# alessandroragano/nomad

Measured on AMD Instinct MI355X. Metric: clips/sec embedded + NxM NOMAD distances, 16kHz x 4s batches, higher is better.
Workload: dtype f32; 1 GPU; configs[1]: batch=256 x 64000 samples (T=199) per GPU, wav2vec2-base + projection head fp32, 224 deg x 32*N ref float64 distances + means; deg_per_gpu=224, ref_total=32, parallelism=clip-sharded x1, all-gather of ref embeddings, collective=none (single process, no process group)

## Files before the change

include/nomad_hip.h:

```cpp
#ifndef NOMAD_HIP_H
#define NOMAD_HIP_H

#include <stddef.h>
#include <stdint.h>

#ifdef __cplusplus
extern "C" {
#endif

#define NOMAD_NUM_LAYERS 12
#define NOMAD_EMBED_DIM 768
#define NOMAD_EMB_DIM 256

typedef enum nomad_status {
    NOMAD_OK = 0,
    NOMAD_ERR_INVALID = -1,
    NOMAD_ERR_NO_DEVICE = -2,
    NOMAD_ERR_HIP = -3,
    NOMAD_ERR_WORKSPACE = -4,
    NOMAD_ERR_IO = -5,
    NOMAD_ERR_FORMAT = -6
} nomad_status;

typedef struct nomad_ctx nomad_ctx;
// ... 145 lines not shown
                              float* emb_dev, void* workspace_dev, size_t workspace_bytes, nomad_stream_t stream);

typedef struct nomad_wav_info {
    int sample_rate, channels, format_tag, bits;
    long long frames;
    long long data_offset;
} nomad_wav_info;
int nomad_wav_probe(const char* const* paths, int n, nomad_wav_info* info, int* status, int threads);
int nomad_wav_frames_at(const nomad_wav_info* info, int target_rate, long long* frames);
int nomad_wav_read_rows(const char* const* paths, const nomad_wav_info* info, int n, const int* row,
                        float* dst_host, long long stride, int target_rate, int* status, int threads);

enum {
    NOMAD_K_GEMM = 0,
    NOMAD_K_ATTN = 1,
    NOMAD_K_FRONT = 2,
    NOMAD_K_ROW = 3,
    NOMAD_K_PAIR = 4,
    NOMAD_K_GEMM_BIG = 5,
    NOMAD_K_GEMM_FINE = 6,
    NOMAD_K_COUNT = 7
};
int nomad_profile_enable(nomad_ctx* ctx, int on);
int nomad_profile_reset(nomad_ctx* ctx);
int nomad_profile_read(nomad_ctx* ctx, double ms[NOMAD_K_COUNT], long long launches[NOMAD_K_COUNT],
                       double flops[NOMAD_K_COUNT]);

int nomad_diag_gemm(nomad_ctx* ctx, const float* A_dev, const float* W_dev, const float* bias_dev,
                    const float* R_dev, float* C_dev, int M, int N, int K, int gelu, int tile,
                    nomad_stream_t stream);
int nomad_diag_gemm_bf16(nomad_ctx* ctx, const void* A_dev, const void* W_dev, const float* bias_dev,
                         const void* R_dev, void* C_dev, int M, int N, int K, int gelu, int tile,
                         nomad_stream_t stream);
int nomad_diag_split_bf16(nomad_ctx* ctx, const float* in_dev, void* out_dev, long long plane, long long n, int inverse,
                          nomad_stream_t stream);
int nomad_diag_gemm_bf16x3(nomad_ctx* ctx, const void* A_dev, const void* W_dev, const float* bias_dev,
                           const void* R_dev, void* C_dev, int M, int N, int K, int gelu, int out_f32,
                           nomad_stream_t stream);
int nomad_diag_attention_bf16x3(nomad_ctx* ctx, const void* qkv_dev, void* out_dev, int B, int T, int waves,
                                nomad_stream_t stream);
int nomad_diag_attention_bf16(nomad_ctx* ctx, const void* qkv_dev, void* out_dev, int B, int T, int q_has_log2e,
                              nomad_stream_t stream);
int nomad_diag_clock_probe(nomad_ctx* ctx, unsigned long long spin_ticks, unsigned long long* out_dev,
                           nomad_stream_t stream);
int nomad_diag_layernorm(nomad_ctx* ctx, const float* in_dev, const float* gamma_dev, const float* beta_dev,
                         float* out_dev, int M, int N, nomad_stream_t stream);
int nomad_diag_attention(nomad_ctx* ctx, const float* qkv_dev, float* out_dev, int B, int T, nomad_stream_t stream);
int nomad_diag_layernorm_bwd(nomad_ctx* ctx, const float* x_dev, const float* g_dev, const float* gamma_dev,
                             float* dx_dev, int M, int N, nomad_stream_t stream);
int nomad_diag_attention_bwd(nomad_ctx* ctx, const float* qkv_dev, const float* dctx_dev, float* ctx_out_dev,
                             float* lse_dev, float* dqkv_dev, int B, int T, nomad_stream_t stream);
int nomad_diag_keep_intermediates(nomad_ctx* ctx, int on);
int nomad_diag_workspace_region(const nomad_ctx* ctx, int B, int n_samples, const char* name,
                                size_t* offset, size_t* bytes);

#ifdef __cplusplus
}
#endif
#endif
```

nomad_amd/_lib.py:

```python
from __future__ import annotations

import ctypes as C
import os

NUM_LAYERS = 12
K_GEMM, K_ATTN, K_FRONT, K_ROW, K_PAIR, K_GEMM_BIG, K_GEMM_FINE, K_COUNT = 0, 1, 2, 3, 4, 5, 6, 7
KERNEL_CLASS_NAMES = ("gemm_mfma_all", "attention_mfma", "frontend", "rowwise", "pairwise_f64",
                      "gemm_mfma_256x128", "gemm_mfma_128x64")

_fp = C.c_void_p


class LayerWeights(C.Structure):
    _fields_ = [(n, _fp) for n in ("q_w", "q_b", "k_w", "k_b", "v_w", "v_b", "o_w", "o_b", "ln1_w", "ln1_b",
                                   "fc1_w", "fc1_b", "fc2_w", "fc2_b", "ln2_w", "ln2_b")]


class Weights(C.Structure):
    _fields_ = ([("conv_w", _fp * 7)] +
                [(n, _fp) for n in ("gn_w", "gn_b", "feat_ln_w", "feat_ln_b", "proj_w", "proj_b",
                                    "pos_v", "pos_g", "pos_b", "enc_ln_w", "enc_ln_b")] +
                [("layers", LayerWeights * NUM_LAYERS), ("emb_w", _fp), ("emb_b", _fp)])


# ... 58 lines not shown
    "nomad_train_enable": (C.c_int, [C.c_void_p, C.POINTER(Weights)]),
    "nomad_train_workspace_bytes": (C.c_int, [C.c_void_p, C.c_int, C.c_int, C.POINTER(C.c_size_t)]),
    "nomad_train_zero_grad": (C.c_int, [C.c_void_p, _fp]),
    "nomad_train_backward": (C.c_int, [C.c_void_p, _fp, C.c_int, C.c_int, _fp, _fp, C.c_size_t, _fp, _fp, C.c_size_t, _fp]),
    "nomad_triplet_loss": (C.c_int, [C.c_void_p, _fp, _fp, _fp, C.c_int, C.c_float, _fp, _fp, _fp, _fp, _fp]),
    "nomad_train_adam_step": (C.c_int, [C.c_void_p, C.c_float, C.c_float, C.c_double, C.c_double, C.c_float, _fp]),
    "nomad_train_read": (C.c_int, [C.c_void_p, C.c_int, _fp, _fp]),
    "nomad_train_write": (C.c_int, [C.c_void_p, C.c_int, _fp, _fp]),
    "nomad_train_set_step": (C.c_int, [C.c_void_p, C.c_longlong]),
    "nomad_train_set_frozen": (C.c_int, [C.c_void_p, C.c_int]),
    "nomad_train_set_convnet": (C.c_int, [C.c_void_p, C.c_int]),
    "nomad_train_set_branches": (C.c_int, [C.c_void_p, C.c_int, C.POINTER(C.c_uint)]),
    "nomad_train_set_stochastic": (C.c_int, [C.c_void_p, C.c_float, C.c_float, C.c_float, C.c_ulonglong, C.c_uint]),
    "nomad_enable_bf16": (C.c_int, [C.c_void_p]),
    "nomad_workspace_bytes_bf16": (C.c_int, [C.c_void_p, C.c_int, C.c_int, C.POINTER(C.c_size_t)]),
    "nomad_embed_bf16": (C.c_int, [C.c_void_p, _fp, C.c_int, C.c_int, _fp, _fp, C.c_size_t, _fp]),
    "nomad_workspace_bytes_ragged_bf16": (C.c_int, [C.c_void_p, C.c_int, C.POINTER(C.c_int), C.POINTER(C.c_size_t)]),
    "nomad_embed_ragged_bf16": (C.c_int, [C.c_void_p, _fp, C.c_int, C.c_int, C.POINTER(C.c_int), _fp, _fp, C.c_size_t, _fp]),
    "nomad_enable_bf16x3": (C.c_int, [C.c_void_p]),
    "nomad_workspace_bytes_bf16x3": (C.c_int, [C.c_void_p, C.c_int, C.c_int, C.POINTER(C.c_size_t)]),
    "nomad_embed_bf16x3": (C.c_int, [C.c_void_p, _fp, C.c_int, C.c_int, _fp, _fp, C.c_size_t, _fp]),
    "nomad_embed_layers_bf16x3": (C.c_int, [C.c_void_p, _fp, C.c_int, C.c_int, _fp, _fp, _fp, _fp, _fp, C.c_size_t, _fp]),
    "nomad_workspace_bytes_ragged_bf16x3": (C.c_int, [C.c_void_p, C.c_int, C.POINTER(C.c_int), C.POINTER(C.c_size_t)]),
    "nomad_embed_ragged_bf16x3": (C.c_int, [C.c_void_p, _fp, C.c_int, C.c_int, C.POINTER(C.c_int), _fp, _fp, C.c_size_t, _fp]),
    "nomad_diag_attention_bf16x3": (C.c_int, [C.c_void_p, _fp, _fp, C.c_int, C.c_int, C.c_int, _fp]),
    "nomad_diag_split_bf16": (C.c_int, [C.c_void_p, _fp, _fp, C.c_longlong, C.c_longlong, C.c_int, _fp]),
    "nomad_diag_gemm_bf16x3": (C.c_int, [C.c_void_p, _fp, _fp, _fp, _fp, _fp, C.c_int, C.c_int, C.c_int, C.c_int, C.c_int, _fp]),
    "nomad_diag_gemm_bf16": (C.c_int, [C.c_void_p, _fp, _fp, _fp, _fp, _fp, C.c_int, C.c_int, C.c_int, C.c_int, C.c_int, _fp]),
    "nomad_diag_attention_bf16": (C.c_int, [C.c_void_p, _fp, _fp, C.c_int, C.c_int, C.c_int, _fp]),
    "nomad_profile_enable": (C.c_int, [C.c_void_p, C.c_int]),
    "nomad_profile_reset": (C.c_int, [C.c_void_p]),
    "nomad_profile_read": (C.c_int, [C.c_void_p, C.POINTER(C.c_double), C.POINTER(C.c_longlong), C.POINTER(C.c_double)]),
    "nomad_diag_gemm": (C.c_int, [C.c_void_p, _fp, _fp, _fp, _fp, _fp, C.c_int, C.c_int, C.c_int, C.c_int, C.c_int, _fp]),
    "nomad_diag_clock_probe": (C.c_int, [C.c_void_p, C.c_ulonglong, _fp, _fp]),
    "nomad_diag_layernorm": (C.c_int, [C.c_void_p, _fp, _fp, _fp, _fp, C.c_int, C.c_int, _fp]),
    "nomad_diag_attention": (C.c_int, [C.c_void_p, _fp, _fp, C.c_int, C.c_int, _fp]),
    "nomad_diag_layernorm_bwd": (C.c_int, [C.c_void_p, _fp, _fp, _fp, _fp, C.c_int, C.c_int, _fp]),
    "nomad_diag_attention_bwd": (C.c_int, [C.c_void_p, _fp, _fp, _fp, _fp, _fp, C.c_int, C.c_int, _fp]),
    "nomad_diag_keep_intermediates": (C.c_int, [C.c_void_p, C.c_int]),
    "nomad_diag_workspace_region": (C.c_int, [C.c_void_p, C.c_int, C.c_int, C.c_char_p,
                                              C.POINTER(C.c_size_t), C.POINTER(C.c_size_t)]),
}

LIB_PATH = os.path.join(os.path.dirname(os.path.abspath(__file__)), "libnomad_hip.so")
DIAG_LIB_PATH = os.path.join(os.path.dirname(os.path.abspath(__file__)), "libnomad_diag.so")
_libs = {}


ABI_VERSION = 3


def load(diag=None):
    if diag is None:
        diag = os.environ.get("NOMAD_DIAG_LIB", "0") == "1"
    diag = bool(diag)
    if diag in _libs:
        return _libs[diag]
    path = DIAG_LIB_PATH if diag else LIB_PATH
    variant = os.environ.get("NOMAD_LIB_VARIANT")
    if variant and variant != "main":
        path = path[:-3] + f"_{variant}.so"
    if not os.path.isfile(path):
        raise RuntimeError(f"{path} is missing: build it with `python -m nomad_amd.build` "
                           "(hipcc --offload-arch=gfx950). nomad_amd has no CPU or PyTorch fallback path.")
    lib = C.CDLL(path)
    for name, (res, args) in SIGNATURES.items():
# ... 24 lines not shown
```

nomad_amd/csrc/nomad_ctx.hip.h:

```cpp
#pragma once
#include <hip/hip_runtime.h>

#include <algorithm>
#include <cmath>
#include <cstdarg>
#include <cstdio>
#include <cstdlib>
#include <cstring>
#include <atomic>
#include <mutex>
#include <string>
#include <vector>

#include "../../include/nomad_hip.h"

#include "dtypes.hip.h"
#include "gemm_f32.hip.h"

#define NOMAD_INTERNAL __attribute__((visibility("hidden")))

using namespace nomad;

inline thread_local char g_err[512] = "";

// ... 14 lines not shown
    } while (0)

constexpr int kConvK[7] = {10, 3, 3, 3, 3, 2, 2};
constexpr int kConvS[7] = {5, 2, 2, 2, 2, 2, 2};
constexpr int kSplitKLayersMaxM = 4096;
constexpr size_t kSplitKPartFloats = (size_t)4 * 512 * 64 * 64;
constexpr long long kPairScratchDoubles = 1 << 21;
constexpr int kCdistMaxD = 4096;
constexpr int kEventChunk = 8192;
const int* const kNoInts = nullptr;
const hipStream_t kNoStream = reinterpret_cast<hipStream_t>(~uintptr_t(0));

}

struct LayerDev {
    float *qkv_w, *qkv_b, *o_w, *o_b, *ln1_w, *ln1_b, *fc1_w, *fc1_b, *fc2_w, *fc2_b, *ln2_w, *ln2_b;
};


struct Tuning {
    bool splitk_lnb_fuse = true;
    bool splitk_ln_fuse = true;
    bool splitk_posconv = true;
    bool splitk_layers = true;
    bool f32_plain_epi = true;
    bool f32_lean = true, f32_direct_epi = true, f32_skew = true, f32_res_ahead = true;
    int f32_mixed = 1;
    int f32_mixed_m1 = 0;
    int f32_mixed_slots = 0;
    double f32_mixed_min = 0.05, f32_mixed_max = 0.70;
    bool f32_mixed_prefer = false;
    bool f32_quant_tile = true;
    bool f32_conv_wino = true;
    double f32_quant_penalty = 0.0;
    bool f32_longk_33 = false;
    int f32_mid_tile = 31;
    bool f32_attn_vt4 = true;
    bool f32_attn_struct_loads = false;
    bool bf16_posconv_slab = true;
    int bf16_attn_dma = 2;
    int bf16_attn_v3 = 2;
    int bf16_attn_tail = 0;
    int bf16_ln_rows = 4;
    bool bf16_conv0_mfma = true;
    bool bf16_conv0_gelu_erf = false;
    int p8_min_tiles = 256;
    bool p8_nt_stores = true;
    int p8_rpre = 3;
    bool x3_plain_epi = true;
    bool p8_three_b = true;
    int p8_n192 = 0;
    bool p9 = true;
    bool p9_res = true;
    bool p9_share = false;
    bool p9_tail_split = false;
    int p9_short = 1;
    bool attn_bwd_small = true;
    bool p9_wl = false;
    bool p9_late = true;
    int p9_skew = 0;
    int concurrent_parts = 1;
};

#ifdef NOMAD_DIAG
static void tuning_from_env(Tuning& t) {
    auto geti = [](const char* n, int d) { const char* e = getenv(n); return e ? atoi(e) : d; };
    auto getb = [](const char* n, bool d) { const char* e = getenv(n); return e ? atoi(e) != 0 : d; };
    auto getd = [](const char* n, double d) { const char* e = getenv(n); return e ? atof(e) : d; };
    t.splitk_ln_fuse = getb("NOMAD_SPLITK_LN", t.splitk_ln_fuse);
    t.splitk_posconv = getb("NOMAD_SPLITK_POSCONV", t.splitk_posconv);
    t.splitk_layers = getb("NOMAD_SPLITK_LAYERS", t.splitk_layers);
    t.f32_plain_epi = getb("NOMAD_F32_PLAIN_EPI", t.f32_plain_epi);
    t.f32_lean = getb("NOMAD_F32_LEAN", t.f32_lean);
    t.f32_direct_epi = getb("NOMAD_F32_DIRECT_EPI", t.f32_direct_epi);
    t.f32_skew = getb("NOMAD_F32_SKEW", t.f32_skew);
    t.f32_res_ahead = getb("NOMAD_F32_RES_AHEAD", t.f32_res_ahead);
    t.f32_mixed = geti("NOMAD_F32_MIXED", t.f32_mixed);
    t.f32_mixed_m1 = geti("NOMAD_F32_MIXED_M1", t.f32_mixed_m1);
    t.f32_mixed_slots = geti("NOMAD_F32_MIXED_SLOTS", t.f32_mixed_slots);
    t.f32_mixed_min = getd("NOMAD_F32_MIXED_MIN", t.f32_mixed_min);
    t.f32_mixed_max = getd("NOMAD_F32_MIXED_MAX", t.f32_mixed_max);
    t.f32_mixed_prefer = getb("NOMAD_F32_MIXED_PREFER", t.f32_mixed_prefer);
    t.f32_quant_tile = getb("NOMAD_F32_QUANT_TILE", t.f32_quant_tile);
    t.f32_conv_wino = getb("NOMAD_F32_CONV_WINO", t.f32_conv_wino);
    t.f32_quant_penalty = getd("NOMAD_F32_QUANT_PENALTY", t.f32_quant_penalty);
    t.f32_longk_33 = getb("NOMAD_F32_LONGK_33", t.f32_longk_33);
    t.f32_mid_tile = geti("NOMAD_F32_MID_TILE", t.f32_mid_tile);
    t.bf16_attn_dma = geti("NOMAD_BF16_ATTN_DMA", t.bf16_attn_dma);
    t.f32_attn_struct_loads = geti("NOMAD_F32_ATTN_STRUCT_LOADS", t.f32_attn_struct_loads) != 0;
    t.bf16_posconv_slab = geti("NOMAD_BF16_POSCONV_SLAB", t.bf16_posconv_slab) != 0;
    t.bf16_attn_v3 = geti("NOMAD_BF16_ATTN_V3", t.bf16_attn_v3);
    t.bf16_attn_tail = geti("NOMAD_BF16_ATTN_TAIL", t.bf16_attn_tail);
    t.bf16_ln_rows = geti("NOMAD_BF16_LN_ROWS", t.bf16_ln_rows);
    t.bf16_conv0_mfma = getb("NOMAD_BF16_CONV0_MFMA", t.bf16_conv0_mfma);
    t.p8_min_tiles = geti("NOMAD_BF16_8PHASE_MIN_TILES", t.p8_min_tiles);
    t.p8_nt_stores = getb("NOMAD_BF16_NT_STORES", t.p8_nt_stores);
    t.p8_rpre = geti("NOMAD_BF16_RPRE", t.p8_rpre);
    t.x3_plain_epi = getb("NOMAD_X3_PLAIN_EPI", t.x3_plain_epi);
    t.p8_three_b = getb("NOMAD_BF16_B3", t.p8_three_b);
    t.p8_n192 = geti("NOMAD_BF16_N192", t.p8_n192);
    t.p9 = getb("NOMAD_BF16_P9", t.p9);
    t.p9_tail_split = getb("NOMAD_BF16_P9_TAIL", t.p9_tail_split);
    t.p9_share = getb("NOMAD_BF16_P9_SHARE", t.p9_share);
    t.p9_res = getb("NOMAD_BF16_P9_RES", t.p9_res);
    t.p9_short = geti("NOMAD_BF16_P9_SHORT", t.p9_short);
    t.p9_skew = geti("NOMAD_BF16_P9_SKEW", t.p9_skew);
    t.p9_late = getb("NOMAD_BF16_P9_LATE", t.p9_late);
    t.p9_wl = getb("NOMAD_BF16_P9_WL", t.p9_wl);
    t.splitk_lnb_fuse = getb("NOMAD_SPLITK_LNB", t.splitk_lnb_fuse);
    t.f32_attn_vt4 = getb("NOMAD_F32_ATTN_VT4", t.f32_attn_vt4);
    t.bf16_conv0_gelu_erf = getb("NOMAD_BF16_CONV0_GELU_ERF", t.bf16_conv0_gelu_erf);
    t.attn_bwd_small = getb("NOMAD_ATTN_BWD_SMALL", t.attn_bwd_small);
}
#endif

struct nomad_ctx {
    int device = 0;
    int num_cus = 256;
    Tuning tune;
    bool keep = false;
    float* conv0_w = nullptr;
    float* conv_w[7] = {};
    float *gn_w = nullptr, *gn_b = nullptr, *fln_w = nullptr, *fln_b = nullptr;
    float *proj_w = nullptr, *proj_b = nullptr;
    float *pos_w = nullptr, *pos_b = nullptr;
    float *eln_w = nullptr, *eln_b = nullptr;
    LayerDev layers[NOMAD_NUM_LAYERS] = {};
    float *emb_w = nullptr, *emb_b = nullptr;
    float* splitk_part = nullptr;
    float* splitk_cur = nullptr;
    size_t splitk_cur_floats = 0;
    bool splitk_ok = false;
    struct PendingLn {
        const float* gamma = nullptr;
        const float* beta = nullptr;
        float* out = nullptr;
        float* out2 = nullptr;
        bool armed = false, done = false;
    } pending_ln;
    struct PendingLnBwd {
        const float* x = nullptr;
        const float* g2 = nullptr;
        const float* gamma = nullptr;
        float* out = nullptr;
        bool armed = false, done = false;
    } pending_lnb;
    std::vector<std::pair<hipStream_t, double*>> pair_scratch;
    std::mutex pair_mu;
    bool bwd_ready = false;
    float* conv_bw_even[7] = {};
    float* conv_bw_odd[7] = {};
    float* conv_bw2[7] = {};
    float* proj_wT = nullptr;
    float* pos_wb = nullptr;
    float *qkv_wT[NOMAD_NUM_LAYERS] = {}, *o_wT[NOMAD_NUM_LAYERS] = {}, *fc1_wT[NOMAD_NUM_LAYERS] = {},
          *fc2_wT[NOMAD_NUM_LAYERS] = {};
    bool bf16_ready = false;
    bf16_t* conv_w16[7] = {};
// ... 88 lines not shown
}

GemmParams dense(const float* A, int lda, const float* W, const float* bias, const float* R, float* C, int M, int N,
                 int K, int gelu) {
    GemmParams p{};
    p.A = A;
    p.amap = plain_map(M, lda);
    p.kchunk = K;
    p.kstride = 0;
    p.W = W;
    p.ldw = K;
    p.C = C;
    p.cmap = plain_map(M, N);
    p.bias = bias;
    p.R = R;
    p.rmap = plain_map(M, N);
    p.M = M;
    p.N = N;
    p.K = K;
    p.n_valid = N;
    p.gelu = gelu;
    return p;
}

}

NOMAD_INTERNAL int run_gemm(nomad_ctx* c, GemmParams p, int groups, int tile, hipStream_t s, int occ = 0);
NOMAD_INTERNAL int gemm_f32_dispatch(nomad_ctx* c, GemmParams p, int groups, int tile, hipStream_t s, int occ);
NOMAD_INTERNAL hipError_t gemm_f32_n48_split(const GemmParams& q, int groups, hipStream_t s, int S);
NOMAD_INTERNAL int pick_tile(const nomad_ctx* c, int M, int N, int K);
NOMAD_INTERNAL int mixed_split_rows(const nomad_ctx* c, int M, int N);
NOMAD_INTERNAL int run_conv_s2_f32(nomad_ctx* c, const float* X, const float* W, float* Y, float* Upre, int B, int Lin, int L,
                                   const int* pp, const int* opref, const int* ipref, int pairs, hipStream_t s);
NOMAD_INTERNAL int run_gemm_bf16(nomad_ctx* c, GemmParams p, int groups, hipStream_t s, int tile = -1);
#ifdef NOMAD_DIAG
NOMAD_INTERNAL int gemm_f32_timeline_read(unsigned long long* out_host, int n);
NOMAD_INTERNAL int gemm_bf16_timeline_read(unsigned long long* out_host, int n);
#endif
```

nomad_amd/csrc/nomad_gemm_f32.hip:

```cpp
#include "nomad_ctx.hip.h"
#include "conv_s2_f32.hip.h"

int gemm_f32_dispatch(nomad_ctx* c, GemmParams p, int groups, int tile, hipStream_t s, int occ) {
    if (tile == 29 && occ == 0) occ = 4;
    const double flops = 2.0 * p.M * (double)p.n_valid * p.K * groups;
    Scope sc(c, s, NOMAD_K_GEMM, flops, tile == 33 ? NOMAD_K_GEMM_BIG : ((tile == 34 || tile == 31 || tile == 48) ? NOMAD_K_GEMM_FINE : -1));
    hipError_t e;
    if (c->gemm_x3 && tile == 48 && p.N == 64)
        tile = 37;
    if (c->gemm_x3 && (tile == 31 || tile == 34 || tile == 37) && p.N % 128 == 0 &&
        (long long)((p.M + 127) / 128) * (p.N / 128) >= 512)
        tile = 20;
    const bool plain_cr = c->tune.f32_plain_epi && p.c_colblk == 0 && p.cmap.clip_rows >= p.M && !p.cmap.pref &&
                          (!p.R || (p.rmap.clip_rows >= p.M && !p.rmap.pref)) && (!p.DG || (p.dgmap.clip_rows >= p.M && !p.dgmap.pref));
    if (c->gemm_x3 && plain_cr && (tile == 20 || tile == 31 || tile == 34 || tile == 37)) {
        constexpr int T = 16 | 32;
        switch (tile) {
            case 20: e = launch_gemm_glds<128, 128, 32, 2, 2, 2, false, 12 | T, true>(p, groups, s, occ_pad(occ, GldsCfg<128, 128, 32, 2, 2>::LDS_BYTES)); break;
            case 31: e = launch_gemm_glds<128, 128, 32, 4, 2, 2, false, 12 | T, true>(p, groups, s, occ_pad(occ, GldsCfg<128, 128, 32, 4, 2>::LDS_BYTES)); break;
            case 34: e = launch_gemm_glds<128, 64, 32, 4, 2, 3, false, 12 | T, true>(p, groups, s); break;
            default: e = launch_gemm_glds<64, 64, 32, 2, 2, 3, false, 12 | T, true>(p, groups, s); break;
        }
        if (e != hipSuccess) return fail(NOMAD_ERR_HIP, "gemm (bf16x3 products) launch: %s", hipGetErrorString(e));
        return 0;
    }
    if (c->gemm_x3 && (tile == 20 || tile == 31 || tile == 33 || tile == 34 || tile == 37)) {
        switch (tile) {
            case 20: e = launch_gemm_glds<128, 128, 32, 2, 2, 2, false, 12, true>(p, groups, s, occ_pad(occ, GldsCfg<128, 128, 32, 2, 2>::LDS_BYTES)); break;
            case 31: e = launch_gemm_glds<128, 128, 32, 4, 2, 2, false, 12, true>(p, groups, s, occ_pad(occ, GldsCfg<128, 128, 32, 4, 2>::LDS_BYTES)); break;
            case 33: e = launch_gemm_glds<256, 128, 16, 4, 2, 3, false, 13, true>(p, groups, s); break;
            case 34: e = launch_gemm_glds<128, 64, 32, 4, 2, 3, false, 12, true>(p, groups, s); break;
            default: e = launch_gemm_glds<64, 64, 32, 2, 2, 3, false, 12, true>(p, groups, s); break;
        }
        if (e != hipSuccess) return fail(NOMAD_ERR_HIP, "gemm (bf16x3 products) launch: %s", hipGetErrorString(e));
// ... 289 lines not shown
    p.pairs = pairs;
    p.tiles_m = (pairs + ConvS2Cfg::BMP - 1) / ConvS2Cfg::BMP;
    p.nclips = B;
    if (ipref) {
        p.pp = pp;
        p.opref = opref;
        p.ipref = ipref;
    } else {
        p.L = L;
        p.Lin = Lin;
        p.ppc = (L + 1) / 2;
        if (Lin < 2 * L + 1 || pairs != B * p.ppc) return fail(NOMAD_ERR_INVALID, "conv_s2: %d clips of %d -> %d frames, %d pairs", B, Lin, L, pairs);
        p.ppc_magic = 0;
        p.ppc_shift = 0;
        if (B > 1 && p.ppc > 1) fast_div_magic((unsigned)p.ppc, &p.ppc_magic, &p.ppc_shift);
    }
    const double flops = 2.0 * (double)pairs * 512 * 2560;
    Scope sc(c, s, NOMAD_K_GEMM, flops, NOMAD_K_GEMM_BIG);
    static LdsAttrOnce attr_u, attr_r;
    hipError_t e;
    if (ipref) {
        if ((e = attr_r.ensure(reinterpret_cast<const void*>(conv_s2_f32_kernel<true>), ConvS2Cfg::LDS_BYTES)) != hipSuccess)
            return fail(NOMAD_ERR_HIP, "conv_s2 attribute: %s", hipGetErrorString(e));
        hipLaunchKernelGGL(conv_s2_f32_kernel<true>, dim3(p.tiles_m * 4), dim3(ConvS2Cfg::NT), ConvS2Cfg::LDS_BYTES, s, p);
    } else {
        if ((e = attr_u.ensure(reinterpret_cast<const void*>(conv_s2_f32_kernel<false>), ConvS2Cfg::LDS_BYTES)) != hipSuccess)
            return fail(NOMAD_ERR_HIP, "conv_s2 attribute: %s", hipGetErrorString(e));
        hipLaunchKernelGGL(conv_s2_f32_kernel<false>, dim3(p.tiles_m * 4), dim3(ConvS2Cfg::NT), ConvS2Cfg::LDS_BYTES, s, p);
    }
    if ((e = hipGetLastError()) != hipSuccess) return fail(NOMAD_ERR_HIP, "conv_s2 launch: %s", hipGetErrorString(e));
    return 0;
}

#ifdef NOMAD_DIAG
extern "C" {
int nomad_diag_conv_s2(nomad_ctx* c, const float* X, const float* W, float* Y, float* U, int B, const int* lin_host, int ragged,
                       void* stream) {
    if (!c || !X || !W || !Y || !lin_host || B <= 0) return fail(NOMAD_ERR_INVALID, "nomad_diag_conv_s2: bad argument");
    std::vector<int> meta(3 * (size_t)(B + 1), 0);
    for (int b = 0; b < B; ++b) {
        const int lin = lin_host[b], L = lin >= 3 ? (lin - 3) / 2 + 1 : 0;
        if (L <= 0 || (!ragged && lin != lin_host[0])) return fail(NOMAD_ERR_INVALID, "nomad_diag_conv_s2: clip %d of %d frames", b, lin);
        meta[b + 1] = meta[b] + (L + 1) / 2;
        meta[(B + 1) + b + 1] = meta[(B + 1) + b] + L;
        meta[2 * (B + 1) + b + 1] = meta[2 * (B + 1) + b] + lin;
    }
    hipStream_t s = static_cast<hipStream_t>(stream);
    int* d = nullptr;
    HIP_TRY(hipMalloc(&d, sizeof(int) * meta.size()));
    int rc = 0;
    if (hipMemcpy(d, meta.data(), sizeof(int) * meta.size(), hipMemcpyHostToDevice) != hipSuccess) rc = fail(NOMAD_ERR_HIP, "nomad_diag_conv_s2: copy");
    const int lin0 = lin_host[0], L0 = (lin0 - 3) / 2 + 1;
    if (rc == 0)
        rc = ragged ? run_conv_s2_f32(c, X, W, Y, U, B, 0, 0, d, d + (B + 1), d + 2 * (B + 1), meta[B], s)
                    : run_conv_s2_f32(c, X, W, Y, U, B, lin0, L0, nullptr, nullptr, nullptr, meta[B], s);
    if (rc == 0 && hipStreamSynchronize(s) != hipSuccess) rc = fail(NOMAD_ERR_HIP, "nomad_diag_conv_s2: kernel");
    (void)hipFree(d);
    return rc;
}
}
#endif
```

nomad_amd/csrc/nomad_hip.hip:

```cpp
#include "nomad_ctx.hip.h"

#include "attention.hip.h"
#include "attention_bf16_v2.hip.h"
#include "attention_bf16_v3.hip.h"
#include "posconv_bf16_slab.hip.h"
#include "attention_f32_v2.hip.h"
#include "attention_bwd.hip.h"
#include "backward.hip.h"
#include "frontend.hip.h"
#include "gemm_bf16.hip.h"
#include "gemm_bf16_8phase.hip.h"
#include "gemm_bf16_p9.hip.h"
#include "gemm_bf16x3.hip.h"
#include "gemm_f32.hip.h"
#ifdef NOMAD_DIAG
#endif
#include "pairwise.hip.h"
#include "rowops.hip.h"
#include "train.hip.h"
#include "wav_reader.h"

namespace {

struct Shapes {
// ... 737 lines not shown
    };
    up(w->conv_w[0], 512 * 10, &c->conv0_w);
    for (int i = 1; i < 7 && rc == 0; ++i) {
        const int k = kConvK[i];
        std::vector<float> r((size_t)512 * k * 512);
        for (int n = 0; n < 512; ++n)
            for (int ci = 0; ci < 512; ++ci)
                for (int t = 0; t < k; ++t) r[(size_t)n * k * 512 + t * 512 + ci] = w->conv_w[i][((size_t)n * 512 + ci) * k + t];
        up(r.data(), r.size(), &c->conv_w[i]);
    }
    up(w->gn_w, 512, &c->gn_w);
    up(w->gn_b, 512, &c->gn_b);
    up(w->feat_ln_w, 512, &c->fln_w);
    up(w->feat_ln_b, 512, &c->fln_b);
    up(w->proj_w, 768 * 512, &c->proj_w);
    up(w->proj_b, 768, &c->proj_b);
    if (rc == 0) {
        std::vector<double> nrm(128, 0.0);
        for (size_t o = 0; o < 768; ++o)
            for (size_t ci = 0; ci < 48; ++ci)
                for (size_t t = 0; t < 128; ++t) {
                    const double v = w->pos_v[(o * 48 + ci) * 128 + t];
                    nrm[t] += v * v;
                }
        std::vector<float> sc(128);
        for (int t = 0; t < 128; ++t) sc[t] = (float)((double)w->pos_g[t] / std::sqrt(nrm[t]));
        std::vector<float> r((size_t)16 * 64 * 6144, 0.f);
        for (size_t g = 0; g < 16; ++g)
            for (size_t n = 0; n < 48; ++n)
                for (size_t ci = 0; ci < 48; ++ci)
                    for (size_t t = 0; t < 128; ++t)
                        r[(g * 64 + n) * 6144 + t * 48 + ci] = w->pos_v[((g * 48 + n) * 48 + ci) * 128 + t] * sc[t];
        up(r.data(), r.size(), &c->pos_w);
    }
    up(w->pos_b, 768, &c->pos_b);
    up(w->enc_ln_w, 768, &c->eln_w);
    up(w->enc_ln_b, 768, &c->eln_b);
    for (int l = 0; l < NOMAD_NUM_LAYERS && rc == 0; ++l) {
        const nomad_layer_weights& lw = w->layers[l];
        LayerDev& d = c->layers[l];
        std::vector<float> qkv((size_t)2304 * 768), qb(2304);
        for (size_t i = 0; i < (size_t)768 * 768; ++i) {
            qkv[i] = lw.q_w[i] * 0.125f;
            qkv[(size_t)768 * 768 + i] = lw.k_w[i];
            qkv[(size_t)2 * 768 * 768 + i] = lw.v_w[i];
        }
        for (int i = 0; i < 768; ++i) {
            qb[i] = lw.q_b[i] * 0.125f;
            qb[768 + i] = lw.k_b[i];
            qb[1536 + i] = lw.v_b[i];
        }
        up(qkv.data(), qkv.size(), &d.qkv_w);
        up(qb.data(), qb.size(), &d.qkv_b);
        up(lw.o_w, 768 * 768, &d.o_w);
        up(lw.o_b, 768, &d.o_b);
        up(lw.ln1_w, 768, &d.ln1_w);
        up(lw.ln1_b, 768, &d.ln1_b);
        up(lw.fc1_w, (size_t)3072 * 768, &d.fc1_w);
        up(lw.fc1_b, 3072, &d.fc1_b);
        up(lw.fc2_w, (size_t)768 * 3072, &d.fc2_w);
        up(lw.fc2_b, 768, &d.fc2_b);
        up(lw.ln2_w, 768, &d.ln2_w);
        up(lw.ln2_b, 768, &d.ln2_b);
    }
    up(w->emb_w, 256 * 768, &c->emb_w);
    up(w->emb_b, 256, &c->emb_b);
// ... 149 lines not shown
        GemmParams p = dense(bf.featln, 512, c->proj_w, c->proj_b, nullptr, xpad, M, 768, 512, 0);
        p.cmap = g.pad_map;
        p.c_colblk = 48;
        p.c_colblk_stride = g.grp_stride;
        if ((rc = run_gemm(c, p, 1, pick_tile(c, M, 768, 512), s))) return rc;
    }
    if (d_in.threshold) {
        Scope sc(c, s, NOMAD_K_ROW, 0.0);
        hipLaunchKernelGGL(dropout_groups_kernel, dim3(M), dim3(192), 0, s, xpad, T, g.grp_stride, d_in, kSiteInput, g.pref[6], g.ppref, B);
    }
    {
        GemmParams p{};
        p.A = xpad;
        p.amap = g.pos_amap;
        p.a_goff = g.grp_stride;
        p.K = 6144;
        p.kchunk = 6144;
        p.W = c->pos_w;
        p.ldw = 6144;
        p.w_goff = 64LL * 6144;
        p.bias = c->pos_b;
        p.bias_goff = 48;
        p.C = sv ? sv->y0 : bf.y;
        p.Upre = sv ? sv->upc : nullptr;
        p.cmap = plain_map(M, 768);
        p.c_goff = 48;
        p.R = xpad;
        p.rmap = g.pad_map;
        p.r_goff = g.grp_stride;
        p.M = M;
        p.N = 64;
        p.n_valid = 48;
        p.gelu = 1;
        if ((rc = run_gemm(c, p, 16, 48, s))) return rc;
    }
    float* x = bf.x;
    float* x2 = bf.x2;
    float* y = bf.y;
    if ((rc = run_layernorm(c, sv ? sv->y0 : y, c->eln_w, c->eln_b, x, nullptr, M, 768, s))) return rc;
    if (d_res.threshold && (rc = run_dropout(c, x, nullptr, x, act, d_res, kSiteEncoder, s))) return rc;

    auto run_layer = [&](int l, int c0, int nc) -> int {
        const LayerDev& d = c->layers[l];
        const long long r0 = g.clip_row0(c0);
        const int Ms = nc == B ? M : (int)(g.clip_row0(c0 + nc) - r0);
        const long long acts = (long long)Ms * 768;
        float* xs = x + r0 * 768;
        float* x2s = x2 + r0 * 768;
        float* hs = bf.h + r0 * 3072;
        float* qkv = (sv ? sv->L[l].qkv : bf.qkv) + r0 * 2304;
        float* ctxb = (sv ? sv->L[l].ctx : bf.ctxb) + r0 * 768;
        float* y1 = (sv ? sv->L[l].y1 : y) + r0 * 768;
        float* y2 = (sv ? sv->L[l].y2 : y) + r0 * 768;
        float* lse = sv ? sv->L[l].lse + 12 * r0 : nullptr;
        float* lo = layers_out ? layers_out + (size_t)l * M * 768 + r0 * 768 : nullptr;
        const unsigned long long idx0 = (unsigned long long)r0 * 768;
        int rc;
        if ((rc = run_gemm(c, dense(xs, 768, d.qkv_w, d.qkv_b, nullptr, qkv, Ms, 2304, 768, 0), 1, pick_tile(c, Ms, 2304, 768), s)))
            return rc;
        if (g.ragged() ? (rc = run_attention(c, g, qkv - r0 * 2304, ctxb - r0 * 768, lse ? lse - 12 * r0 : nullptr, s, &d_att, site_attn(l), c0, nc))
                       : (rc = run_attention(c, g, qkv, ctxb, lse, s, &d_att, site_attn(l), c0, nc)))
            return rc;
        auto arm_ln = [&](const float* g_, const float* b_, float* out_, float* out2_) {
            c->pending_ln = {};
            if (!c->tune.splitk_ln_fuse || d_res.threshold) return;
            c->pending_ln.gamma = g_;
            c->pending_ln.beta = b_;
// ... 1644 lines not shown
        v.push_back({fe + "0.2.weight", o.gn_w, 512});
        v.push_back({fe + "0.2.bias", o.gn_b, 512});
        for (int i = 1; i < 7; ++i) v.push_back({fe + std::to_string(i) + ".0.weight", o.conv_w[i], (size_t)512 * 512 * kConvK[i]});
        v.push_back({"embedding_layer.1.weight", o.emb_w, 256 * 768});
        v.push_back({"embedding_layer.1.bias", o.emb_b, 256});
        return v;
    }();
    return segs;
}

void rebuild_conv_bwd_weights(nomad_ctx* c, hipStream_t s) {
    auto transpose = [&](const float* in, int ld_in, float* out, int ld_out, int R, int C) {
        hipLaunchKernelGGL(transpose_kernel, dim3((C + 31) / 32, (R + 31) / 32), dim3(32, 8), 0, s, in, ld_in, out, ld_out, R, C);
    };
    for (int i = 1; i <= 4; ++i) {
        transpose(c->conv_w[i] + 2 * 512, 1536, c->conv_bw_even[i], 1024, 512, 512);
        transpose(c->conv_w[i], 1536, c->conv_bw_even[i] + 512, 1024, 512, 512);
        transpose(c->conv_w[i] + 512, 1536, c->conv_bw_odd[i], 512, 512, 512);
    }
    for (int i = 5; i <= 6; ++i)
        transpose(c->conv_w[i], 1024, c->conv_bw2[i], 512, 512, 1024);
}

int refresh_weights(nomad_ctx* c, hipStream_t s) {
    const ParamOffsets po = make_param_offsets();
    auto transpose = [&](const float* in, int ld_in, float* out, int ld_out, int R, int C) {
        hipLaunchKernelGGL(transpose_kernel, dim3((C + 31) / 32, (R + 31) / 32), dim3(32, 8), 0, s, in, ld_in, out, ld_out, R, C);
    };
    hipLaunchKernelGGL(tap_dot_partial_kernel, dim3(576), dim3(256), 0, s, c->theta + po.pos_v, (const float*)nullptr,
                       c->tap_partial);
    hipLaunchKernelGGL(tap_sum_final_kernel, dim3(1), dim3(1024), 0, s, c->tap_partial, 576, c->pos_nrm2);
    hipLaunchKernelGGL(posconv_fold_kernel, dim3(768), dim3(256), 0, s, c->theta + po.pos_v, c->theta + po.pos_g,
                       c->pos_nrm2, c->pos_w);
    hipLaunchKernelGGL(posconv_bwd_weight_kernel, dim3(16 * 64), dim3(256), 0, s, c->pos_w, c->pos_wb);
    transpose(c->proj_w, 512, c->proj_wT, 768, 768, 512);
    for (int i = 1; i < 7; ++i) {
        const long long n = 512LL * 512 * kConvK[i];
        hipLaunchKernelGGL(conv_repack_kernel, dim3((unsigned)((n + 255) / 256)), dim3(256), 0, s, c->theta + po.conv_w[i], c->conv_w[i],
                           kConvK[i]);
    }
    rebuild_conv_bwd_weights(c, s);
    for (int l = 0; l < NOMAD_NUM_LAYERS; ++l) {
        const LayerDev& d = c->layers[l];
        const LayerOffsets& lo = po.L[l];
        const long long w4 = (long long)2304 * 768 / 4, q4 = (long long)768 * 768 / 4;
        hipLaunchKernelGGL(scale_rows_kernel, dim3((unsigned)((w4 + 255) / 256)), dim3(256), 0, s,
                           reinterpret_cast<const float4*>(c->theta + lo.qkv_w), reinterpret_cast<float4*>(d.qkv_w), w4, q4, 0.125f);
        hipLaunchKernelGGL(scale_rows_kernel, dim3(3), dim3(256), 0, s, reinterpret_cast<const float4*>(c->theta + lo.qkv_b),
                           reinterpret_cast<float4*>(d.qkv_b), 576LL, 192LL, 0.125f);
        transpose(d.qkv_w, 768, c->qkv_wT[l], 2304, 2304, 768);
        transpose(d.o_w, 768, c->o_wT[l], 768, 768, 768);
        transpose(d.fc1_w, 768, c->fc1_wT[l], 3072, 3072, 768);
        transpose(d.fc2_w, 3072, c->fc2_wT[l], 768, 768, 3072);
    }
    HIP_TRY(hipGetLastError());
    c->bf16_ready = false;
    c->x3_ready = false;
    return 0;
}

}

extern "C" {

int nomad_set_gemm_precision(nomad_ctx* c, int mode) {
    if (!c || (mode != 0 && mode != 1)) return fail(NOMAD_ERR_INVALID, "nomad_set_gemm_precision: mode must be 0 (fp32 MFMA) or 1 (bf16x3 products)");
// ... 519 lines not shown
```

Before: 2488 clips/s.

## Add slab-based MFMA kernel for positional convolution with fragment-ordered weights

Replaces the generic im2col-style GEMM for the 128-tap grouped positional convolution with a dedicated kernel. Each block loads a contiguous slab of padded input frames into LDS once, then iterates over only the valid taps per 16-row tile using f32 MFMA with weights pre-permuted into fragment order. It fuses bias, GELU and the residual add. This removes redundant reads of overlapping input windows and skips taps that fall entirely in padding, at the cost of a new weight buffer, extra setup kernels, and an LDS-heavy launch that may limit occupancy.

```diff
diff --git a/include/nomad_hip.h b/include/nomad_hip.h
--- a/include/nomad_hip.h
+++ b/include/nomad_hip.h
@@ -201,6 +201,9 @@
 int nomad_diag_gemm_bf16(nomad_ctx* ctx, const void* A_dev, const void* W_dev, const float* bias_dev,
                          const void* R_dev, void* C_dev, int M, int N, int K, int gelu, int tile,
                          nomad_stream_t stream);
+int nomad_diag_posconv_f32(nomad_ctx* ctx, const float* xpad_dev, float* y_dev, int B, int T, const int* lens_host,
+                           nomad_stream_t stream, int variant);
+int nomad_diag_posconv_f32_taps(int T, int t0s, int* lo, int* hi);
 int nomad_diag_split_bf16(nomad_ctx* ctx, const float* in_dev, void* out_dev, long long plane, long long n, int inverse,
                           nomad_stream_t stream);
 int nomad_diag_gemm_bf16x3(nomad_ctx* ctx, const void* A_dev, const void* W_dev, const float* bias_dev,
diff --git a/nomad_amd/_lib.py b/nomad_amd/_lib.py
--- a/nomad_amd/_lib.py
+++ b/nomad_amd/_lib.py
@@ -114,6 +114,8 @@
     "nomad_profile_reset": (C.c_int, [C.c_void_p]),
     "nomad_profile_read": (C.c_int, [C.c_void_p, C.POINTER(C.c_double), C.POINTER(C.c_longlong), C.POINTER(C.c_double)]),
     "nomad_diag_gemm": (C.c_int, [C.c_void_p, _fp, _fp, _fp, _fp, _fp, C.c_int, C.c_int, C.c_int, C.c_int, C.c_int, _fp]),
+    "nomad_diag_posconv_f32": (C.c_int, [C.c_void_p, _fp, _fp, C.c_int, C.c_int, C.POINTER(C.c_int), _fp, C.c_int]),
+    "nomad_diag_posconv_f32_taps": (C.c_int, [C.c_int, C.c_int, C.POINTER(C.c_int), C.POINTER(C.c_int)]),
     "nomad_diag_clock_probe": (C.c_int, [C.c_void_p, C.c_ulonglong, _fp, _fp]),
     "nomad_diag_layernorm": (C.c_int, [C.c_void_p, _fp, _fp, _fp, _fp, C.c_int, C.c_int, _fp]),
     "nomad_diag_attention": (C.c_int, [C.c_void_p, _fp, _fp, C.c_int, C.c_int, _fp]),
diff --git a/nomad_amd/csrc/nomad_ctx.hip.h b/nomad_amd/csrc/nomad_ctx.hip.h
--- a/nomad_amd/csrc/nomad_ctx.hip.h
+++ b/nomad_amd/csrc/nomad_ctx.hip.h
@@ -70,6 +70,7 @@
     bool f32_mixed_prefer = false;
     bool f32_quant_tile = true;
     bool f32_conv_wino = true;
+    bool f32_posconv_slab = true;
     double f32_quant_penalty = 0.0;
     bool f32_longk_33 = false;
     int f32_mid_tile = 31;
@@ -121,6 +122,7 @@
     t.f32_mixed_prefer = getb("NOMAD_F32_MIXED_PREFER", t.f32_mixed_prefer);
     t.f32_quant_tile = getb("NOMAD_F32_QUANT_TILE", t.f32_quant_tile);
     t.f32_conv_wino = getb("NOMAD_F32_CONV_WINO", t.f32_conv_wino);
+    t.f32_posconv_slab = getb("NOMAD_F32_POSCONV_SLAB", t.f32_posconv_slab);
     t.f32_quant_penalty = getd("NOMAD_F32_QUANT_PENALTY", t.f32_quant_penalty);
     t.f32_longk_33 = getb("NOMAD_F32_LONGK_33", t.f32_longk_33);
     t.f32_mid_tile = geti("NOMAD_F32_MID_TILE", t.f32_mid_tile);
@@ -162,6 +164,7 @@
     float *gn_w = nullptr, *gn_b = nullptr, *fln_w = nullptr, *fln_b = nullptr;
     float *proj_w = nullptr, *proj_b = nullptr;
     float *pos_w = nullptr, *pos_b = nullptr;
+    float* pos_wfrag = nullptr;
     float *eln_w = nullptr, *eln_b = nullptr;
     LayerDev layers[NOMAD_NUM_LAYERS] = {};
     float *emb_w = nullptr, *emb_b = nullptr;
@@ -316,6 +319,9 @@
 NOMAD_INTERNAL int mixed_split_rows(const nomad_ctx* c, int M, int N);
 NOMAD_INTERNAL int run_conv_s2_f32(nomad_ctx* c, const float* X, const float* W, float* Y, float* Upre, int B, int Lin, int L,
                                    const int* pp, const int* opref, const int* ipref, int pairs, hipStream_t s);
+NOMAD_INTERNAL int run_posconv_f32_slab(nomad_ctx* c, const float* xpad, float* y, int max_t, int B, long long M, const int* tpref,
+                                        const int* ppref, hipStream_t s);
+NOMAD_INTERNAL int posconv_f32_wfrag_build(nomad_ctx* c, hipStream_t s);
 NOMAD_INTERNAL int run_gemm_bf16(nomad_ctx* c, GemmParams p, int groups, hipStream_t s, int tile = -1);
 #ifdef NOMAD_DIAG
 NOMAD_INTERNAL int gemm_f32_timeline_read(unsigned long long* out_host, int n);
diff --git a/nomad_amd/csrc/nomad_gemm_f32.hip b/nomad_amd/csrc/nomad_gemm_f32.hip
--- a/nomad_amd/csrc/nomad_gemm_f32.hip
+++ b/nomad_amd/csrc/nomad_gemm_f32.hip
@@ -1,5 +1,6 @@
 #include "nomad_ctx.hip.h"
 #include "conv_s2_f32.hip.h"
+#include "posconv_f32_slab.hip.h"
 
 int gemm_f32_dispatch(nomad_ctx* c, GemmParams p, int groups, int tile, hipStream_t s, int occ) {
     if (tile == 29 && occ == 0) occ = 4;
@@ -355,6 +356,97 @@
     return 0;
 }
 
+int posconv_f32_wfrag_build(nomad_ctx* c, hipStream_t s) {
+    if (!c->pos_wfrag) {
+        void* d = nullptr;
+        HIP_TRY(hipMalloc(&d, posconv_f32_wfrag_elems() * sizeof(float)));
+        c->allocs.push_back(d);
+        c->pos_wfrag = static_cast<float*>(d);
+    }
+    hipLaunchKernelGGL(posconv_f32_wfrag_kernel, dim3(16 * 384), dim3(192), 0, s, c->pos_w, c->pos_wfrag);
+    HIP_TRY(hipGetLastError());
+    if (!s) HIP_TRY(hipStreamSynchronize(nullptr));
+    return 0;
+}
+
+int run_posconv_f32_slab(nomad_ctx* c, const float* xpad, float* y, int max_t, int B, long long M, const int* tpref, const int* ppref,
+                         hipStream_t s) {
+    if (!c->pos_wfrag) return fail(NOMAD_ERR_INVALID, "posconv_f32_slab: no fragment-ordered weights");
+    Scope sc(c, s, NOMAD_K_GEMM, 2.0 * (double)M * 768.0 * 6144.0, NOMAD_K_GEMM_FINE);
+    HIP_TRY(launch_posconv_f32_slab(xpad, c->pos_wfrag, c->pos_b, y, max_t, B, tpref, ppref, s));
+    return 0;
+}
+
+extern "C" {
+int nomad_diag_posconv_f32(nomad_ctx* c, const float* xpad, float* y, int B, int T, const int* lens_host, nomad_stream_t stream, int variant) {
+    if (!c || !xpad || !y || B <= 0 || (!lens_host && T <= 0) || (variant != 0 && variant != 1) || c->gemm_x3)
+        return fail(NOMAD_ERR_INVALID, "nomad_diag_posconv_f32: bad argument");
+    hipStream_t s = static_cast<hipStream_t>(stream);
+    std::vector<int> meta(2 * (size_t)(B + 1), 0);
+    int max_t = T;
+    if (lens_host) {
+        max_t = 0;
+        for (int b = 0; b < B; ++b) {
+            if (lens_host[b] <= 0) return fail(NOMAD_ERR_INVALID, "nomad_diag_posconv_f32: clip %d of %d frames", b, lens_host[b]);
+            meta[b + 1] = meta[b] + lens_host[b];
+            meta[(B + 1) + b + 1] = meta[(B + 1) + b] + lens_host[b] + 128;
+            max_t = lens_host[b] > max_t ? lens_host[b] : max_t;
+        }
+    }
+    const long long M = lens_host ? meta[B] : (long long)B * T;
+    const long long pad_rows = lens_host ? meta[2 * B + 1] : (long long)B * (T + 128);
+    int* d = nullptr;
+    if (lens_host) {
+        HIP_TRY(hipMalloc(&d, sizeof(int) * meta.size()));
+        if (hipMemcpy(d, meta.data(), sizeof(int) * meta.size(), hipMemcpyHostToDevice) != hipSuccess) {
+            (void)hipFree(d);
+            return fail(NOMAD_ERR_HIP, "nomad_diag_posconv_f32: copy");
+        }
+    }
+    const int *tpref = d, *ppref = d ? d + (B + 1) : nullptr;
+    int rc;
+    if (variant == 1) {
+        rc = run_posconv_f32_slab(c, xpad, y, max_t, B, M, tpref, ppref, s);
+    } else {
+        GemmParams p{};
+        p.A = xpad;
+        p.amap = lens_host ? RowMap{0, 0, 0, 48, tpref, ppref, B, 48} : RowMap{0, (long long)(T + 128) * 48, T, 48};
+        p.a_goff = pad_rows * 48;
+        p.K = 6144;
+        p.kchunk = 6144;
+        p.W = c->pos_w;
+        p.ldw = 6144;
+        p.w_goff = 64LL * 6144;
+        p.bias = c->pos_b;
+        p.bias_goff = 48;
+        p.C = y;
+        p.cmap = plain_map((int)M, 768);
+        p.c_goff = 48;
+        p.R = xpad;
+        p.rmap = lens_host ? RowMap{64LL * 48, 0, 0, 48, tpref, ppref, B, 48} : RowMap{64LL * 48, (long long)(T + 128) * 48, T, 48};
+        p.r_goff = pad_rows * 48;
+        p.M = (int)M;
+        p.N = 64;
+        p.n_valid = 48;
+        p.gelu = 1;
+        rc = run_gemm(c, p, 16, 48, s);
+    }
+    if (d) {
+        if (rc == 0 && hipStreamSynchronize(s) != hipSuccess) rc = fail(NOMAD_ERR_HIP, "nomad_diag_posconv_f32: kernel");
+        (void)hipFree(d);
+    }
+    return rc;
+}
+
+int nomad_diag_posconv_f32_taps(int T, int t0s, int* lo, int* hi) {
+    if (!lo || !hi || T <= 0) return fail(NOMAD_ERR_INVALID, "nomad_diag_posconv_f32_taps: bad argument");
+    const PosTaps r = posconv_f32_taps(T, t0s);
+    *lo = r.lo;
+    *hi = r.hi;
+    return 0;
+}
+}
+
 #ifdef NOMAD_DIAG
 extern "C" {
 int nomad_diag_conv_s2(nomad_ctx* c, const float* X, const float* W, float* Y, float* U, int B, const int* lin_host, int ragged,
diff --git a/nomad_amd/csrc/nomad_hip.hip b/nomad_amd/csrc/nomad_hip.hip
--- a/nomad_amd/csrc/nomad_hip.hip
+++ b/nomad_amd/csrc/nomad_hip.hip
@@ -793,6 +793,7 @@
                     for (size_t t = 0; t < 128; ++t)
                         r[(g * 64 + n) * 6144 + t * 48 + ci] = w->pos_v[((g * 48 + n) * 48 + ci) * 128 + t] * sc[t];
         up(r.data(), r.size(), &c->pos_w);
+        if (rc == 0) rc = posconv_f32_wfrag_build(c, nullptr);
     }
     up(w->pos_b, 768, &c->pos_b);
     up(w->enc_ln_w, 768, &c->eln_w);
@@ -1008,7 +1009,9 @@
         p.N = 64;
         p.n_valid = 48;
         p.gelu = 1;
-        if ((rc = run_gemm(c, p, 16, 48, s))) return rc;
+        if (!sv && !c->gemm_x3 && c->tune.f32_posconv_slab && !posconv_splitk_applies(c, p, 16, 48)) {
+            if ((rc = run_posconv_f32_slab(c, xpad, bf.y, g.max_t, B, M, g.pref[6], g.ppref, s))) return rc;
+        } else if ((rc = run_gemm(c, p, 16, 48, s))) return rc;
     }
     float* x = bf.x;
     float* x2 = bf.x2;
@@ -2719,6 +2722,7 @@
     hipLaunchKernelGGL(tap_sum_final_kernel, dim3(1), dim3(1024), 0, s, c->tap_partial, 576, c->pos_nrm2);
     hipLaunchKernelGGL(posconv_fold_kernel, dim3(768), dim3(256), 0, s, c->theta + po.pos_v, c->theta + po.pos_g,
                        c->pos_nrm2, c->pos_w);
+    if (int rc = posconv_f32_wfrag_build(c, s)) return rc;
     hipLaunchKernelGGL(posconv_bwd_weight_kernel, dim3(16 * 64), dim3(256), 0, s, c->pos_w, c->pos_wb);
     transpose(c->proj_w, 512, c->proj_wT, 768, 768, 512);
     for (int i = 1; i < 7; ++i) {
diff --git a/nomad_amd/csrc/posconv_f32_slab.hip.h b/nomad_amd/csrc/posconv_f32_slab.hip.h
--- /dev/null
+++ b/nomad_amd/csrc/posconv_f32_slab.hip.h
@@ -0,0 +1,168 @@
+#pragma once
+#include <hip/hip_runtime.h>
+
+#include "dtypes.hip.h"
+#include "gemm_f32.hip.h"
+
+namespace nomad {
+
+constexpr int kPosSlabRows = 256;
+constexpr int kPosSlabWaves = 8;
+
+struct PosTaps {
+    int lo, hi;
+};
+__host__ __device__ inline PosTaps posconv_f32_taps(int T, int t0s) {
+    if (t0s < 0 || t0s >= T) return PosTaps{1, 0};
+    const int t1s = t0s + 15 < T ? t0s + 15 : T - 1;
+    PosTaps r;
+    r.lo = 64 - t1s > 0 ? 64 - t1s : 0;
+    r.hi = T + 63 - t0s < 127 ? T + 63 - t0s : 127;
+    return r;
+}
+
+constexpr int posconv_f32_slab_lds(int rows16) { return ((rows16 + 127) * 192 + 1023) & ~1023; }
+
+__global__ __launch_bounds__(192) void posconv_f32_wfrag_kernel(const float* __restrict__ w , float* __restrict__ wfrag) {
+    const int g = blockIdx.x / 384, kg = blockIdx.x - g * 384;
+    const int j = threadIdx.x >> 6, lane = threadIdx.x & 63;
+    const f32x4 v = *reinterpret_cast<const f32x4*>(w + ((long long)g * 64 + 16 * j + (lane & 15)) * 6144 + 16 * kg + 4 * (lane >> 4));
+    *reinterpret_cast<f32x4*>(wfrag + (((long long)g * 384 + kg) * 3 + j) * 256 + lane * 4) = v;
+}
+constexpr size_t posconv_f32_wfrag_elems() { return (size_t)16 * 384 * 3 * 256; }
+
+template <int MASK>
+__device__ __forceinline__ void posconv_f32_taps_run(f32x4 (&acc)[2][3], const float* __restrict__ slab, const char* __restrict__ wg,
+                                                     unsigned wlane, const int (&ap)[2], int tap0, int tap1) {
+    f32x4 w[3][3], a[3][2];
+    const int kg_last = 3 * tap1 + 2;
+    auto ldw = [&](int kg, int j) { return *reinterpret_cast<const f32x4*>(wg + (wlane + (unsigned)kg * 3072u + (unsigned)j * 1024u)); };
+    auto lda = [&](int kg, int i) { return *reinterpret_cast<const f32x4*>(slab + ap[i] + 16 * kg); };
+#pragma unroll
+    for (int q = 0; q < 3; ++q) {
+#pragma unroll
+        for (int j = 0; j < 3; ++j) w[q][j] = ldw(3 * tap0 + q, j);
+        __builtin_amdgcn_sched_barrier(0);
+    }
+#pragma unroll
+    for (int q = 0; q < 2; ++q) {
+#pragma unroll
+        for (int i = 0; i < 2; ++i)
+            if (MASK >> i & 1) a[q][i] = lda(3 * tap0 + q, i);
+        __builtin_amdgcn_sched_barrier(0);
+    }
+#pragma unroll 1
+    for (int tap = tap0; tap <= tap1; ++tap) {
+        const int tn = tap < tap1 ? tap + 1 : tap1;
+#pragma unroll
+        for (int q = 0; q < 3; ++q) {
+            const int ka = 3 * tap + q + 2 < kg_last ? 3 * tap + q + 2 : kg_last;
+#pragma unroll
+            for (int i = 0; i < 2; ++i)
+                if (MASK >> i & 1) a[(q + 2) % 3][i] = lda(ka, i);
+            __builtin_amdgcn_sched_barrier(0);
+#pragma unroll
+            for (int c = 0; c < 4; ++c)
+#pragma unroll
+                for (int i = 0; i < 2; ++i)
+                    if (MASK >> i & 1) {
+#pragma unroll
+                        for (int j = 0; j < 3; ++j) acc[i][j] = __builtin_amdgcn_mfma_f32_16x16x4f32(w[q][j][c], a[q][i][c], acc[i][j], 0, 0, 0);
+                    }
+            __builtin_amdgcn_sched_barrier(0);
+#pragma unroll
+            for (int j = 0; j < 3; ++j) w[q][j] = ldw(3 * tn + q, j);
+            __builtin_amdgcn_sched_barrier(0);
+        }
+    }
+}
+
+__global__ __launch_bounds__(64 * kPosSlabWaves, 4) void posconv_f32_slab_kernel(const float* __restrict__ xpad, const float* __restrict__ wfrag,
+                                                                                 const float* __restrict__ bias, float* __restrict__ y,
+                                                                                 int T_uniform, int B, int nchunks,
+                                                                                 const int* __restrict__ tpref, const int* __restrict__ ppref) {
+    extern __shared__ __attribute__((aligned(16))) float pcs_lds[];
+    const int g = blockIdx.y;
+    const int b = (int)blockIdx.x / nchunks, t0 = ((int)blockIdx.x - b * nchunks) * kPosSlabRows;
+    const int T = tpref ? tpref[b + 1] - tpref[b] : T_uniform;
+    if (t0 >= T) return;
+    const long long row0 = tpref ? (long long)tpref[b] : (long long)b * T_uniform;
+    const long long pad0 = tpref ? (long long)ppref[b] : (long long)b * (T_uniform + 128);
+    const long long grp_frames = tpref ? (long long)ppref[B] : (long long)B * (T_uniform + 128);
+    const int tid = threadIdx.x, lane = tid & 63;
+    const int wave = __builtin_amdgcn_readfirstlane(tid >> 6), nwaves = (int)blockDim.x >> 6;
+    const int fr = lane & 15, fq = lane >> 4;
+
+    const int rc = T - t0 < kPosSlabRows ? T - t0 : kPosSlabRows;
+    const int valid = (rc + 127) * 192;
+    {
+        const float* src = uniform_ptr(xpad + (g * grp_frames + pad0 + t0) * 48);
+        const __amdgpu_buffer_rsrc_t rsrc = __builtin_amdgcn_make_buffer_rsrc(const_cast<float*>(src), 0, valid, 0x00020000);
+        for (int blk = wave; blk * 1024 < valid; blk += nwaves) {
+            int off = blk * 1024 + lane * 16;
+            off = off < valid ? off : valid - 16;
+            __builtin_amdgcn_raw_ptr_buffer_load_lds(rsrc, (lptr_t)(pcs_lds + blk * 256), 16, off, 0, 0, 0);
+        }
+    }
+    f32x4 acc[2][3];
+#pragma unroll
+    for (int i = 0; i < 2; ++i)
+#pragma unroll
+        for (int j = 0; j < 3; ++j) acc[i][j] = (f32x4){0.f, 0.f, 0.f, 0.f};
+    asm volatile("s_waitcnt vmcnt(0)" ::: "memory");
+    __syncthreads();
+
+    const int ta = t0 + 16 * wave, tb = ta + 16 * kPosSlabWaves;
+    const PosTaps ra = posconv_f32_taps(T, ta);
+    if (ra.lo > ra.hi) return;
+    const PosTaps rb = tb < t0 + kPosSlabRows ? posconv_f32_taps(T, tb) : PosTaps{1, 0};
+    const char* wg = reinterpret_cast<const char*>(wfrag + (long long)g * 384 * 3 * 256);
+    const unsigned wlane = (unsigned)lane * 16u;
+    const int ap[2] = {48 * (16 * wave + fr) + 4 * fq, 48 * (16 * (wave + kPosSlabWaves) + fr) + 4 * fq};
+    if (rb.lo > rb.hi) {
+        posconv_f32_taps_run<1>(acc, pcs_lds, wg, wlane, ap, ra.lo, ra.hi);
+    } else {
+        if (rb.lo < ra.lo) posconv_f32_taps_run<2>(acc, pcs_lds, wg, wlane, ap, rb.lo, ra.lo - 1);
+        posconv_f32_taps_run<3>(acc, pcs_lds, wg, wlane, ap, ra.lo, rb.hi);
+        if (rb.hi < ra.hi) posconv_f32_taps_run<1>(acc, pcs_lds, wg, wlane, ap, rb.hi + 1, ra.hi);
+    }
+
+    f32x4 bq[3];
+#pragma unroll
+    for (int j = 0; j < 3; ++j) bq[j] = *reinterpret_cast<const f32x4*>(bias + g * 48 + 16 * j + 4 * fq);
+#pragma unroll
+    for (int i = 0; i < 2; ++i) {
+        const int tl = 16 * (wave + kPosSlabWaves * i) + fr, t = t0 + tl;
+        if (tl < kPosSlabRows && t < T) {
+            float* dst = y + (row0 + t) * 768 + g * 48 + 4 * fq;
+            const float* res = pcs_lds + (tl + 64) * 48 + 4 * fq;
+#pragma unroll
+            for (int j = 0; j < 3; ++j) {
+                const f32x4 rv = *reinterpret_cast<const f32x4*>(res + 16 * j);
+                f32x4 v;
+#pragma unroll
+                for (int r = 0; r < 4; ++r) {
+                    float u = acc[i][j][r] + bq[j][r];
+                    u = gelu_erf(u);
+                    v[r] = u + rv[r];
+                }
+                *reinterpret_cast<f32x4*>(dst + 16 * j) = v;
+            }
+        }
+    }
+}
+
+inline hipError_t launch_posconv_f32_slab(const float* xpad, const float* wfrag, const float* bias, float* y, int max_t, int B,
+                                          const int* tpref, const int* ppref, hipStream_t s) {
+    static LdsAttrOnce configured;
+    if (hipError_t e = configured.ensure(reinterpret_cast<const void*>(posconv_f32_slab_kernel), posconv_f32_slab_lds(kPosSlabRows)); e != hipSuccess)
+        return e;
+    const int nchunks = (max_t + kPosSlabRows - 1) / kPosSlabRows;
+    const int rows16 = max_t >= kPosSlabRows ? kPosSlabRows : (max_t + 15) & ~15;
+    const int waves = rows16 / 16 < kPosSlabWaves ? rows16 / 16 : kPosSlabWaves;
+    hipLaunchKernelGGL(posconv_f32_slab_kernel, dim3((unsigned)B * nchunks, 16), dim3(64 * waves), posconv_f32_slab_lds(rows16), s, xpad, wfrag,
+                       bias, y, max_t, B, nchunks, tpref, ppref);
+    return hipGetLastError();
+}
+
+}
```

Result: no change. 2496 clips/s (median of 6 runs) (+0.3%).
